# klemens-floege/oneprot

Hardware: AMD Instinct MI355X
Metric: protein-pairs/sec/node (seq+struct-token, L=512, ESM-2-150M) (higher is better)
Workload: dtype bf16; 1 GPU; cfg-2: seq<->struct_token sub-step, facebook/esm2_t30_150M_UR50D / facebook/esm2_t30_150M_UR50D, L=512, 256 pairs/GPU per modality, global batch 256, output_dim 1024, CLIP local_loss+gather_with_grad, L1 0.01, Adam 1e-3, clip 1.0, sequence encoder frozen (reference default), random-init weights; global_batch=256, seq_len=512, parallelism=dp1, frozen_sequence_encoder=True

## Files before the change

oneprot_amd/csrc/gemm_nt_ln.hip:

```cpp
#include "gemm_epi8.h"
#ifndef GLN_X_NT
#define GLN_X_NT 0
#endif

namespace gln {
using g8::gload16; using g8::lane_perm; using g8::as_f; using g8::to_rows_addr; using g8::run_groups;

constexpr int BM = 128, BN = 640, MT = 4, NT = 10, NH = 5;
constexpr int A_UNIT = BM * 128, W_UNIT = 320 * 64;
constexpr int NA = 2, NW = 6;
constexpr int OFF_W = NA * A_UNIT, OFF_S = OFF_W + NW * W_UNIT, LDS = OFF_S + 4096;
constexpr int A_IPW = 2;
static_assert(LDS <= 160 * 1024, "LDS");

struct LnArgs {
  const bf16_t* A; const unsigned char* Wp;
  int M, K, lda;
  const float* bias; const float* resid; float* x_out;
  const float* gamma; const float* beta; float eps;
  bf16_t* h_out; float* mean; float* rstd;
  int tiles;
  int late_ticks;
};

__device__ __forceinline__ void bar() { asm volatile("s_barrier" ::: "memory"); }
template <int N> __device__ __forceinline__ void wait_lgkm() { asm volatile("s_waitcnt lgkmcnt(%0)" ::"n"(N) : "memory"); }
__device__ __forceinline__ void glds16(unsigned voff, const unsigned char* sbase, unsigned lds_dst) {
  unsigned keep;
  asm volatile("s_mov_b32 %0, m0\n\ts_mov_b32 m0, %3\n\ts_nop 0\n\tglobal_load_lds_dwordx4 %1, %2\n\ts_mov_b32 m0, %0"
               : "=&s"(keep) : "v"(voff), "s"(sbase), "s"(lds_dst) : "memory");
}

template <int IMM> __device__ __forceinline__ void gload16s(u32x4& d, unsigned voff, const void* sbase) {
  asm volatile("global_load_dwordx4 %0, %1, %2 offset:%3" : "=v"(d) : "v"(voff), "s"(sbase), "n"(IMM) : "memory");
}

__global__ void __launch_bounds__(256) k_pack_w(const bf16_t* __restrict__ W, int K, u32x4* __restrict__ Wp) {
  const int units = K / 32 * 2;
  for (int idx = blockIdx.x * 256 + threadIdx.x; idx < units * 320 * 4; idx += gridDim.x * 256) {
    const int pos = idx & 3, hr = (idx >> 2) % 320, u = idx / (320 * 4);
    const int k32 = u >> 1, nh = u & 1;
    const int c = pos ^ ((hr >> 1) & 3);
    const int n = (hr / 80) * 160 + nh * 80 + hr % 80;
    Wp[idx] = *reinterpret_cast<const u32x4*>(W + (size_t)n * K + k32 * 32 + c * 8);
  }
}

__global__ void __launch_bounds__(512, 2) k_gemm_ln(const LnArgs p) {
  extern __shared__ __attribute__((aligned(16))) unsigned char smem[];
  const int tid = threadIdx.x, lane = tid & 63;
  const int wave = __builtin_amdgcn_readfirstlane(tid >> 6);
  const int grp = wave >> 2;
  const int wm = wave >> 2, wc = wave & 3;
  const int nk = p.K >> 6;
  const int PH = 4 * nk;
  const int G = gridDim.x;
  const int Q = p.tiles > (int)blockIdx.x ? (p.tiles - (int)blockIdx.x + G - 1) / G : 0;
  if (Q == 0) return;
  const unsigned lds0 = (unsigned)(uintptr_t)LDS_PTR(smem);

  const int sr = lane >> 3, sc = lane & 7;
  unsigned a_voff[A_IPW];
#pragma unroll
  for (int i = 0; i < A_IPW; ++i) {
    const int row = (i * 8 + wave) * 8 + sr;
    a_voff[i] = (unsigned)row * (unsigned)p.lda * 2u + (unsigned)(sc ^ ((row >> 1) & 7)) * 16u;
  }
  const unsigned w_voff = (unsigned)lane * 16u;
  auto issue_a = [&](const unsigned char* abase, int slot) {
#pragma unroll
    for (int i = 0; i < A_IPW; ++i) glds16(a_voff[i], abase, lds0 + slot * A_UNIT + (i * 8 + wave) * 1024);
  };
  auto issue_w = [&](const unsigned char* wbase, int slot) {
#pragma unroll
    for (int i = 0; i < 3; ++i)
      if (i < 2 || wave < 4) glds16(w_voff, wbase + (i * 8 + wave) * 1024, lds0 + OFF_W + slot * W_UNIT + (i * 8 + wave) * 1024);
  };

  int wq = 0, wu = 0, wslot = 0;
  int aq = 0, as = 0, aslot = 0;
  auto a_ptr = [&](int q, int s) { return reinterpret_cast<const unsigned char*>(p.A + (size_t)(((int)blockIdx.x + q * G) * BM) * p.lda) + (size_t)s * 128; };
  auto next_w = [&]() { if (wq < Q) issue_w(p.Wp + (size_t)wu * W_UNIT, wslot); if (++wu == PH) { wu = 0; ++wq; } wslot = wslot + 1 == NW ? 0 : wslot + 1; };
  auto next_a = [&]() { if (aq < Q) issue_a(a_ptr(aq, as), aslot); if (++as == nk) { as = 0; ++aq; } aslot ^= 1; };

  const int fr = lane & 15, fq = lane >> 4;
  const unsigned a_rd = (unsigned)(wm * 64 + fr) * 128u + (unsigned)((fq ^ (fr >> 1)) << 4);
  const unsigned w_rd = OFF_W + (unsigned)(wc * 80 + fr) * 64u + (unsigned)((fq ^ ((fr >> 1) & 3)) << 4);

  f32x4 acc[MT][NT];
  auto zero_acc = [&]() {
    float z = 0.f;
    asm volatile("" : "+v"(z));
#pragma unroll
    for (int i = 0; i < MT; ++i)
#pragma unroll
      for (int j = 0; j < NT; ++j) acc[i][j] = (f32x4){z, z, z, z};
  };
  zero_acc();
  bf8_t fa[MT], fb[NH];

  constexpr int N0 = 4 * 3 + A_IPW, N1 = 4 * 2 + A_IPW;
  int rslot = 0;
  auto phase = [&](auto kkc, auto halfc, int abuf, const bool stores_behind, const bool more) {
    constexpr int KK = decltype(kkc)::value, HALF = decltype(halfc)::value;
    if constexpr (HALF == 0) {
      const unsigned char* ab = smem + abuf * A_UNIT;
#pragma unroll
      for (int mt = 0; mt < MT; ++mt) fa[mt] = *reinterpret_cast<const bf8_t*>(ab + ((a_rd + mt * 2048) ^ (KK << 6)));
      __builtin_amdgcn_sched_barrier(0);
    }
    const unsigned char* wb = smem + rslot * W_UNIT;
#pragma unroll
    for (int nt = 0; nt < NH; ++nt) fb[nt] = *reinterpret_cast<const bf8_t*>(wb + w_rd + nt * 1024);
    __builtin_amdgcn_sched_barrier(0);
    next_w();
    if constexpr (KK == 1 && HALF == 1) next_a();
    wait_lgkm<0>();
    if (!more) wait_vmcnt<0>();
    else if (stores_behind) wait_vmcnt<63>();
    else if (grp == 0) wait_vmcnt<N0>(); else wait_vmcnt<N1>();
    bar();
    __builtin_amdgcn_sched_barrier(0);
    __builtin_amdgcn_s_setprio(1);
#pragma unroll
    for (int mt = 0; mt < MT; ++mt)
#pragma unroll
      for (int nt = 0; nt < NH; ++nt)
        acc[mt][HALF * NH + nt] = __builtin_amdgcn_mfma_f32_16x16x32_bf16(fb[nt], fa[mt], acc[mt][HALF * NH + nt], 0, 0, 0);
    __builtin_amdgcn_s_setprio(0);
    __builtin_amdgcn_sched_barrier(0);
    bar();
    rslot = rslot + 1 == NW ? 0 : rslot + 1;
  };

  next_a();
  for (int i = 0; i < 5; ++i) next_w();
  next_a();
  if (Q * nk < 2) wait_vmcnt<0>();
  else if (grp == 0) wait_vmcnt<N0>(); else wait_vmcnt<N1>();
  bar();

  const int c = lane & 15, q4 = lane >> 4;
  const int rsr = lane >> 2, rsq = lane & 3;
  const int pa = to_rows_addr(lane);
  float* scratch = reinterpret_cast<float*>(smem + OFF_S);
  int abuf = 0;
  long done_phases = 0;
  const long total_phases = (long)Q * PH;
#pragma clang loop unroll(disable)
  for (int q = 0; q < Q; ++q) {
    if (grp == 1) bar();
#pragma clang loop unroll(disable)
    for (int s = 0; s < nk; ++s) {
      const bool sb = q > 0 && s == 0;
      phase(std::integral_constant<int, 0>{}, std::integral_constant<int, 0>{}, abuf, sb, done_phases + 6 <= total_phases); ++done_phases;
      phase(std::integral_constant<int, 0>{}, std::integral_constant<int, 1>{}, abuf, sb, done_phases + 6 <= total_phases); ++done_phases;
      phase(std::integral_constant<int, 1>{}, std::integral_constant<int, 0>{}, abuf, sb, done_phases + 6 <= total_phases); ++done_phases;
      phase(std::integral_constant<int, 1>{}, std::integral_constant<int, 1>{}, abuf, sb, done_phases + 6 <= total_phases); ++done_phases;
      abuf ^= 1;
    }
    if (grp == 0) bar();

    const int m0 = ((int)blockIdx.x + q * G) * BM;
    const size_t o0 = (size_t)(m0 + wm * 64 + rsr) * BN + wc * 160 + rsq * 4;
    const size_t rstep = (size_t)16 * BN;
    const unsigned bias_off = (unsigned)(wc * 160 + q4 * 4) * 4u;
    const unsigned row_off = (unsigned)((wm * 64 + rsr) * BN + wc * 160 + rsq * 4) * 4u;
    const float* res_t = p.resid + (size_t)m0 * BN;
    float* xo = p.x_out + o0;
    float s1[MT] = {0.f, 0.f, 0.f, 0.f};
    {
      constexpr int GL = 2 + 4, GS = 4, NG = (NT / 2) * (MT / 2);
      auto load = [&](auto gc, u32x4 (&r)[GL]) {
        constexpr int g = decltype(gc)::value, a2 = 2 * (g / (MT / 2)), i2 = 2 * (g % (MT / 2));
        gload16s<a2 * 64>(r[0], bias_off, p.bias);
        gload16s<(a2 + 1) * 64>(r[1], bias_off, p.bias);
        gload16s<a2 * 64>(r[2], row_off, res_t + i2 * rstep);
        gload16s<(a2 + 1) * 64>(r[3], row_off, res_t + i2 * rstep);
        gload16s<a2 * 64>(r[4], row_off, res_t + (i2 + 1) * rstep);
        gload16s<(a2 + 1) * 64>(r[5], row_off, res_t + (i2 + 1) * rstep);
      };
      auto finish = [&](auto gc, const u32x4 (&r)[GL]) {
        constexpr int g = decltype(gc)::value, a2 = 2 * (g / (MT / 2)), i2 = 2 * (g % (MT / 2));
        float h0, h1, h2, h3;
        g8::static_for([&](auto uc) {
          constexpr int u = decltype(uc)::value, j = a2 + (u & 1), i = i2 + (u >> 1);
          u32x4 a;
          a.x = __builtin_bit_cast(unsigned, acc[i][j][0] + as_f(r[u & 1].x)); a.y = __builtin_bit_cast(unsigned, acc[i][j][1] + as_f(r[u & 1].y));
          a.z = __builtin_bit_cast(unsigned, acc[i][j][2] + as_f(r[u & 1].z)); a.w = __builtin_bit_cast(unsigned, acc[i][j][3] + as_f(r[u & 1].w));
          a = lane_perm(pa, a);
          const u32x4 t = r[2 + u];
          const float x0 = as_f(a.x) + as_f(t.x), x1 = as_f(a.y) + as_f(t.y), x2 = as_f(a.z) + as_f(t.z), x3 = as_f(a.w) + as_f(t.w);
          acc[i][j] = (f32x4){x0, x1, x2, x3};
          s1[i] += (x0 + x1) + (x2 + x3);
          if constexpr ((u & 1) == 0) { h0 = x0; h1 = x1; h2 = x2; h3 = x3; }
          else {
            __builtin_amdgcn_sched_barrier(0);
            gst(xo + i * rstep + (j - 1) * 16, h0, h1, h2, h3, GLN_X_NT);
            gst(xo + i * rstep + j * 16, x0, x1, x2, x3, GLN_X_NT);
            __builtin_amdgcn_sched_barrier(0);
          }
        }, std::make_integer_sequence<int, 4>{});
      };
      run_groups<NG, GL, GS>(load, finish);
    }
    float mw[MT], m2[MT];
#pragma unroll
    for (int i = 0; i < MT; ++i) {
      float s = s1[i];
      s += __shfl_xor(s, 1, 64); s += __shfl_xor(s, 2, 64);
      mw[i] = s * (1.0f / 160.0f);
      float qv = 0.f;
#pragma unroll
      for (int j = 0; j < NT; ++j) {
        const float a = acc[i][j][0] - mw[i], b = acc[i][j][1] - mw[i], cc = acc[i][j][2] - mw[i], d = acc[i][j][3] - mw[i];
        qv += (a * a + b * b) + (cc * cc + d * d);
      }
      qv += __shfl_xor(qv, 1, 64); qv += __shfl_xor(qv, 2, 64);
      m2[i] = qv;
      if (rsq == 0) *reinterpret_cast<float2*>(scratch + ((wm * 64 + i * 16 + rsr) * 4 + wc) * 2) = make_float2(mw[i], qv);
    }
    asm volatile("s_waitcnt lgkmcnt(0)" ::: "memory");
    bar();
    float mean[MT], rstd[MT];
#pragma unroll
    for (int i = 0; i < MT; ++i) {
      const float4 p01 = *reinterpret_cast<const float4*>(scratch + (wm * 64 + i * 16 + rsr) * 8);
      const float4 p23 = *reinterpret_cast<const float4*>(scratch + (wm * 64 + i * 16 + rsr) * 8 + 4);
      const float mu = ((p01.x + p01.z) + (p23.x + p23.z)) * 0.25f;
      const float d0 = p01.x - mu, d1 = p01.z - mu, d2 = p23.x - mu, d3 = p23.z - mu;
      const float M2 = ((p01.y + p01.w) + (p23.y + p23.w)) + 160.0f * ((d0 * d0 + d1 * d1) + (d2 * d2 + d3 * d3));
      mean[i] = mu;
      rstd[i] = rsqrtf(M2 * (1.0f / 640.0f) + p.eps);
      if (wc == 0 && rsq == 0) {
        if (p.mean) p.mean[m0 + wm * 64 + i * 16 + rsr] = mu;
        if (p.rstd) p.rstd[m0 + wm * 64 + i * 16 + rsr] = rstd[i];
      }
    }
    asm volatile("s_waitcnt lgkmcnt(0)" ::: "memory");
    bar();
    {
      constexpr int GL = 4, GS = MT, NG = NT / 2;
      const unsigned gb_off = (unsigned)(wc * 160 + rsq * 4) * 4u;
      bf16_t* ho = p.h_out + (size_t)(m0 + wm * 64 + rsr) * BN + wc * 160 + (rsq & 1) * 16 + (rsq >> 1) * 8;
      const bool odd = (rsq & 1) != 0;
      auto pass2 = [&](auto oddc) {
        constexpr bool ODDW = decltype(oddc)::value;
        auto load = [&](auto gc, u32x4 (&r)[GL]) {
          constexpr int g = decltype(gc)::value, j = 2 * (ODDW ? g : (g + NG - 1) % NG);
          gload16s<j * 64>(r[0], gb_off, p.gamma); gload16s<j * 64>(r[1], gb_off, p.beta);
          gload16s<(j + 1) * 64>(r[2], gb_off, p.gamma); gload16s<(j + 1) * 64>(r[3], gb_off, p.beta);
        };
        auto finish = [&](auto gc, const u32x4 (&r)[GL]) {
          constexpr int g = decltype(gc)::value, a = ODDW ? g : (g + NG - 1) % NG, j = 2 * a;
#pragma unroll
          for (int i = 0; i < MT; ++i) {
            u32x2 w[2];
#pragma unroll
            for (int t = 0; t < 2; ++t) {
              const u32x4 ga = r[2 * t], be = r[2 * t + 1];
              const float h0 = (acc[i][j + t][0] - mean[i]) * rstd[i] * as_f(ga.x) + as_f(be.x), h1 = (acc[i][j + t][1] - mean[i]) * rstd[i] * as_f(ga.y) + as_f(be.y);
              const float h2 = (acc[i][j + t][2] - mean[i]) * rstd[i] * as_f(ga.z) + as_f(be.z), h3 = (acc[i][j + t][3] - mean[i]) * rstd[i] * as_f(ga.w) + as_f(be.w);
              w[t].x = pack2bf(h0, h1); w[t].y = pack2bf(h2, h3);
            }
            const unsigned sx = odd ? w[0].x : w[1].x, sy = odd ? w[0].y : w[1].y;
            const unsigned rx = (unsigned)__builtin_amdgcn_update_dpp(0, (int)sx, 0xB1, 0xF, 0xF, false);
            const unsigned ry = (unsigned)__builtin_amdgcn_update_dpp(0, (int)sy, 0xB1, 0xF, 0xF, false);
            u32x4 o;
            o.x = odd ? rx : w[0].x; o.y = odd ? ry : w[0].y; o.z = odd ? w[1].x : rx; o.w = odd ? w[1].y : ry;
            gst(reinterpret_cast<u32x4*>(ho + i * rstep + a * 32), o, 0);
          }
        };
        run_groups<NG, GL, GS>(load, finish);
      };
      if (wc & 1) pass2(std::true_type{}); else pass2(std::false_type{});
    }
    zero_acc();
  }
}


namespace g1 {
constexpr int BM = 64, NWU = 3;
constexpr int A_UNIT = BM * 128;
constexpr int OFF_W = NA * A_UNIT, OFF_S = OFF_W + NWU * W_UNIT, LDS = OFF_S + 2048;
static_assert(2 * LDS <= 160 * 1024, "two work-groups per CU");
}

__global__ void __launch_bounds__(256, 2) k_gemm_ln4(const LnArgs p) {
  extern __shared__ __attribute__((aligned(16))) unsigned char smem[];
  const int tid = threadIdx.x, lane = tid & 63;
  const int wave = __builtin_amdgcn_readfirstlane(tid >> 6);
  const int wc = wave;
  const int nk = p.K >> 6;
  const int PH = 4 * nk;
  const int G = gridDim.x;
  const int Q = p.tiles > (int)blockIdx.x ? (p.tiles - (int)blockIdx.x + G - 1) / G : 0;
  if (Q == 0) return;
  const unsigned lds0 = (unsigned)(uintptr_t)LDS_PTR(smem);
  if (p.late_ticks > 0 && (int)blockIdx.x >= (G >> 1)) {
    const long long t0 = (long long)__builtin_amdgcn_s_memrealtime();
    while ((long long)__builtin_amdgcn_s_memrealtime() - t0 < p.late_ticks) __builtin_amdgcn_s_sleep(16);
  }

  const int sr = lane >> 3, sc = lane & 7;
  unsigned a_voff[2];
#pragma unroll
  for (int i = 0; i < 2; ++i) {
    const int row = (i * 4 + wave) * 8 + sr;
    a_voff[i] = (unsigned)row * (unsigned)p.lda * 2u + (unsigned)(sc ^ ((row >> 1) & 7)) * 16u;
  }
  const unsigned w_voff = (unsigned)lane * 16u;
  auto issue_a = [&](const unsigned char* abase, int slot) {
#pragma unroll
    for (int i = 0; i < 2; ++i) glds16(a_voff[i], abase, lds0 + slot * g1::A_UNIT + (i * 4 + wave) * 1024);
  };
  auto issue_w = [&](const unsigned char* wbase, int slot) {
#pragma unroll
    for (int i = 0; i < 5; ++i) glds16(w_voff, wbase + (i * 4 + wave) * 1024, lds0 + g1::OFF_W + slot * W_UNIT + (i * 4 + wave) * 1024);
  };
  int wq = 0, wu = 0, wslot = 0;
  int aq = 0, as = 0, aslot = 0;
  auto a_ptr = [&](int q, int s) { return reinterpret_cast<const unsigned char*>(p.A + (size_t)(((int)blockIdx.x + q * G) * g1::BM) * p.lda) + (size_t)s * 128; };
  auto next_w = [&]() { if (wq < Q) issue_w(p.Wp + (size_t)wu * W_UNIT, wslot); if (++wu == PH) { wu = 0; ++wq; } wslot = wslot + 1 == g1::NWU ? 0 : wslot + 1; };
  auto next_a = [&]() { if (aq < Q) issue_a(a_ptr(aq, as), aslot); if (++as == nk) { as = 0; ++aq; } aslot ^= 1; };

  const int fr = lane & 15, fq = lane >> 4;
  const unsigned a_rd = (unsigned)fr * 128u + (unsigned)((fq ^ (fr >> 1)) << 4);
  const unsigned w_rd = g1::OFF_W + (unsigned)(wc * 80 + fr) * 64u + (unsigned)((fq ^ ((fr >> 1) & 3)) << 4);

  f32x4 acc[MT][NT];
  auto zero_acc = [&]() {
    float z = 0.f;
    asm volatile("" : "+v"(z));
#pragma unroll
    for (int i = 0; i < MT; ++i)
#pragma unroll
      for (int j = 0; j < NT; ++j) acc[i][j] = (f32x4){z, z, z, z};
  };
  zero_acc();
  bf8_t fa[MT], fb[NH];

  int rslot = 0;
  bool skip_w = false;
  auto phase = [&](auto kkc, auto halfc, int abuf, const int tail, const bool a_too) {
    constexpr int KK = decltype(kkc)::value, HALF = decltype(halfc)::value;
    if constexpr (HALF == 0) {
      const unsigned char* ab = smem + abuf * g1::A_UNIT;
#pragma unroll
      for (int mt = 0; mt < MT; ++mt) fa[mt] = *reinterpret_cast<const bf8_t*>(ab + ((a_rd + mt * 2048) ^ (KK << 6)));
    }
    const unsigned char* wb = smem + rslot * W_UNIT;
#pragma unroll
    for (int nt = 0; nt < NH; ++nt) fb[nt] = *reinterpret_cast<const bf8_t*>(wb + w_rd + nt * 1024);
    __builtin_amdgcn_sched_barrier(0);
    if (!skip_w) next_w();
    skip_w = false;
    if (a_too) next_a();
    wait_lgkm<0>();
    __builtin_amdgcn_sched_barrier(0);
    __builtin_amdgcn_s_setprio(1);
#pragma unroll
    for (int mt = 0; mt < MT; ++mt)
#pragma unroll
      for (int nt = 0; nt < NH; ++nt)
        acc[mt][HALF * NH + nt] = __builtin_amdgcn_mfma_f32_16x16x32_bf16(fb[nt], fa[mt], acc[mt][HALF * NH + nt], 0, 0, 0);
    __builtin_amdgcn_s_setprio(0);
    __builtin_amdgcn_sched_barrier(0);
    if (tail == 2) wait_vmcnt<0>();
    else if (tail == 1) wait_vmcnt<63>();
    else if (KK == HALF) wait_vmcnt<5 + 2>(); else wait_vmcnt<5>();
    bar();
    rslot = rslot + 1 == g1::NWU ? 0 : rslot + 1;
  };

  next_a(); next_w(); next_w(); next_a();
  if (Q * nk < 2) wait_vmcnt<0>(); else wait_vmcnt<5 + 2>();
  bar();

  const int c = lane & 15, q4 = lane >> 4;
  const int rsr = lane >> 2, rsq = lane & 3;
  const int pa = to_rows_addr(lane);
  float* scratch = reinterpret_cast<float*>(smem + g1::OFF_S);
  int abuf = 0;
  long done = 0;
  const long total = (long)Q * PH;
  int behind = 0;
#pragma clang loop unroll(disable)
  for (int q = 0; q < Q; ++q) {
#pragma clang loop unroll(disable)
    for (int s = 0; s < nk; ++s) {
      auto tl = [&]() { const int t = done + 8 > total ? 2 : (behind > 0 ? 1 : 0); if (behind > 0) --behind; ++done; return t; };
      { const int t = tl(); phase(std::integral_constant<int, 0>{}, std::integral_constant<int, 0>{}, abuf, t, false); }
      { const int t = tl(); phase(std::integral_constant<int, 0>{}, std::integral_constant<int, 1>{}, abuf, t, false); }
      { const int t = tl(); phase(std::integral_constant<int, 1>{}, std::integral_constant<int, 0>{}, abuf, t, false); }
      { const int t = tl(); phase(std::integral_constant<int, 1>{}, std::integral_constant<int, 1>{}, abuf, t, true); }
      abuf ^= 1;
    }
    if (q + 1 < Q) { next_w(); skip_w = true; behind = 2; }

    const int m0 = ((int)blockIdx.x + q * G) * g1::BM;
    const size_t o0 = (size_t)(m0 + rsr) * BN + wc * 160 + rsq * 4;
    const size_t rstep = (size_t)16 * BN;
    const unsigned bias_off = (unsigned)(wc * 160 + q4 * 4) * 4u;
    const unsigned row_off = (unsigned)(rsr * BN + wc * 160 + rsq * 4) * 4u;
    const float* res_t = p.resid + (size_t)m0 * BN;
    float* xo = p.x_out + o0;
    float s1[MT] = {0.f, 0.f, 0.f, 0.f};
    {
      constexpr int GL = 2 + 4, GS = 4, NG = (NT / 2) * (MT / 2);
      auto load = [&](auto gc, u32x4 (&r)[GL]) {
        constexpr int g = decltype(gc)::value, a2 = 2 * (g / (MT / 2)), i2 = 2 * (g % (MT / 2));
        gload16s<a2 * 64>(r[0], bias_off, p.bias);
        gload16s<(a2 + 1) * 64>(r[1], bias_off, p.bias);
        gload16s<a2 * 64>(r[2], row_off, res_t + i2 * rstep);
        gload16s<(a2 + 1) * 64>(r[3], row_off, res_t + i2 * rstep);
        gload16s<a2 * 64>(r[4], row_off, res_t + (i2 + 1) * rstep);
        gload16s<(a2 + 1) * 64>(r[5], row_off, res_t + (i2 + 1) * rstep);
      };
      auto finish = [&](auto gc, const u32x4 (&r)[GL]) {
        constexpr int g = decltype(gc)::value, a2 = 2 * (g / (MT / 2)), i2 = 2 * (g % (MT / 2));
        float h0, h1, h2, h3;
        g8::static_for([&](auto uc) {
          constexpr int u = decltype(uc)::value, j = a2 + (u & 1), i = i2 + (u >> 1);
          u32x4 a;
          a.x = __builtin_bit_cast(unsigned, acc[i][j][0] + as_f(r[u & 1].x)); a.y = __builtin_bit_cast(unsigned, acc[i][j][1] + as_f(r[u & 1].y));
          a.z = __builtin_bit_cast(unsigned, acc[i][j][2] + as_f(r[u & 1].z)); a.w = __builtin_bit_cast(unsigned, acc[i][j][3] + as_f(r[u & 1].w));
          a = lane_perm(pa, a);
          const u32x4 t = r[2 + u];
          const float x0 = as_f(a.x) + as_f(t.x), x1 = as_f(a.y) + as_f(t.y), x2 = as_f(a.z) + as_f(t.z), x3 = as_f(a.w) + as_f(t.w);
          acc[i][j] = (f32x4){x0, x1, x2, x3};
          s1[i] += (x0 + x1) + (x2 + x3);
          if constexpr ((u & 1) == 0) { h0 = x0; h1 = x1; h2 = x2; h3 = x3; }
          else {
            __builtin_amdgcn_sched_barrier(0);
            gst(xo + i * rstep + (j - 1) * 16, h0, h1, h2, h3, GLN_X_NT);
            gst(xo + i * rstep + j * 16, x0, x1, x2, x3, GLN_X_NT);
            __builtin_amdgcn_sched_barrier(0);
          }
        }, std::make_integer_sequence<int, 4>{});
      };
      run_groups<NG, GL, GS>(load, finish);
    }
    float mw[MT], m2[MT];
#pragma unroll
    for (int i = 0; i < MT; ++i) {
      float s = s1[i];
      s += __shfl_xor(s, 1, 64); s += __shfl_xor(s, 2, 64);
      mw[i] = s * (1.0f / 160.0f);
      float qv = 0.f;
#pragma unroll
      for (int j = 0; j < NT; ++j) {
        const float a = acc[i][j][0] - mw[i], b = acc[i][j][1] - mw[i], cc = acc[i][j][2] - mw[i], d = acc[i][j][3] - mw[i];
        qv += (a * a + b * b) + (cc * cc + d * d);
      }
      qv += __shfl_xor(qv, 1, 64); qv += __shfl_xor(qv, 2, 64);
      m2[i] = qv;
      if (rsq == 0) *reinterpret_cast<float2*>(scratch + ((i * 16 + rsr) * 4 + wc) * 2) = make_float2(mw[i], qv);
    }
    asm volatile("s_waitcnt lgkmcnt(0)" ::: "memory");
    bar();
    float mean[MT], rstd[MT];
#pragma unroll
    for (int i = 0; i < MT; ++i) {
      const float4 p01 = *reinterpret_cast<const float4*>(scratch + (i * 16 + rsr) * 8);
      const float4 p23 = *reinterpret_cast<const float4*>(scratch + (i * 16 + rsr) * 8 + 4);
      const float mu = ((p01.x + p01.z) + (p23.x + p23.z)) * 0.25f;
      const float d0 = p01.x - mu, d1 = p01.z - mu, d2 = p23.x - mu, d3 = p23.z - mu;
      const float M2 = ((p01.y + p01.w) + (p23.y + p23.w)) + 160.0f * ((d0 * d0 + d1 * d1) + (d2 * d2 + d3 * d3));
      mean[i] = mu;
      rstd[i] = rsqrtf(M2 * (1.0f / 640.0f) + p.eps);
      if (wc == 0 && rsq == 0) {
        if (p.mean) p.mean[m0 + i * 16 + rsr] = mu;
        if (p.rstd) p.rstd[m0 + i * 16 + rsr] = rstd[i];
      }
    }
    asm volatile("s_waitcnt lgkmcnt(0)" ::: "memory");
    bar();
    {
      constexpr int GL = 4, GS = MT, NG = NT / 2;
      const unsigned gb_off = (unsigned)(wc * 160 + rsq * 4) * 4u;
      bf16_t* ho = p.h_out + (size_t)(m0 + rsr) * BN + wc * 160 + (rsq & 1) * 16 + (rsq >> 1) * 8;
      const bool odd = (rsq & 1) != 0;
      auto pass2 = [&](auto oddc) {
        constexpr bool ODDW = decltype(oddc)::value;
        auto load = [&](auto gc, u32x4 (&r)[GL]) {
          constexpr int g = decltype(gc)::value, j = 2 * (ODDW ? g : (g + NG - 1) % NG);
          gload16s<j * 64>(r[0], gb_off, p.gamma); gload16s<j * 64>(r[1], gb_off, p.beta);
          gload16s<(j + 1) * 64>(r[2], gb_off, p.gamma); gload16s<(j + 1) * 64>(r[3], gb_off, p.beta);
        };
        auto finish = [&](auto gc, const u32x4 (&r)[GL]) {
          constexpr int g = decltype(gc)::value, a = ODDW ? g : (g + NG - 1) % NG, j = 2 * a;
#pragma unroll
          for (int i = 0; i < MT; ++i) {
            u32x2 w[2];
#pragma unroll
            for (int t = 0; t < 2; ++t) {
              const u32x4 ga = r[2 * t], be = r[2 * t + 1];
              const float h0 = (acc[i][j + t][0] - mean[i]) * rstd[i] * as_f(ga.x) + as_f(be.x), h1 = (acc[i][j + t][1] - mean[i]) * rstd[i] * as_f(ga.y) + as_f(be.y);
              const float h2 = (acc[i][j + t][2] - mean[i]) * rstd[i] * as_f(ga.z) + as_f(be.z), h3 = (acc[i][j + t][3] - mean[i]) * rstd[i] * as_f(ga.w) + as_f(be.w);
              w[t].x = pack2bf(h0, h1); w[t].y = pack2bf(h2, h3);
            }
            const unsigned sx = odd ? w[0].x : w[1].x, sy = odd ? w[0].y : w[1].y;
            const unsigned rx = (unsigned)__builtin_amdgcn_update_dpp(0, (int)sx, 0xB1, 0xF, 0xF, false);
            const unsigned ry = (unsigned)__builtin_amdgcn_update_dpp(0, (int)sy, 0xB1, 0xF, 0xF, false);
            u32x4 o;
            o.x = odd ? rx : w[0].x; o.y = odd ? ry : w[0].y; o.z = odd ? w[1].x : rx; o.w = odd ? w[1].y : ry;
            gst(reinterpret_cast<u32x4*>(ho + i * rstep + a * 32), o, 0);
          }
        };
        run_groups<NG, GL, GS>(load, finish);
      };
      if (wc & 1) pass2(std::true_type{}); else pass2(std::false_type{});
    }
    zero_acc();
  }
}

}

extern "C" int oneprot_gemm_ln_pack_weight(const void* W, void* Wp, int N, int K, void* stream) {
  if (!W || !Wp || N != gln::BN || K <= 0 || (K & 63) || (((uintptr_t)W | (uintptr_t)Wp) & 15)) return OP_EINVAL;
  const int n = K / 32 * 2 * 320 * 4;
  int blocks = (n + 255) / 256; if (blocks > 2048) blocks = 2048;
  hipLaunchKernelGGL(gln::k_pack_w, dim3(blocks), dim3(256), 0, (hipStream_t)stream, (const bf16_t*)W, K, (u32x4*)Wp);
  return launch_status();
}

static int g_gln_form = 0;
extern "C" void oneprot_gemm_ln_form(int form) { g_gln_form = form; }
extern "C" int oneprot_gemm_ln_form_get(void) { return g_gln_form; }

extern "C" int oneprot_gemm_bf16_nt_resid_ln(const void* A, const void* Wp, int64_t M, int N, int K, int lda, const float* bias, const float* resid, float* x_out,
                                             const float* gamma, const float* beta, float eps, void* h_out, float* mean, float* rstd, void* stream) {
  if (!A || !Wp || !bias || !resid || !x_out || !gamma || !beta || !h_out || M <= 0 || M > 0x7fffffff) return OP_EINVAL;
  if (N != gln::BN || (M % gln::BM) || K <= 0 || (K & 63) || (lda & 7) || lda < K || (size_t)gln::BM * lda * 2 >= (1ull << 31)) return OP_EINVAL;
  if (((uintptr_t)A | (uintptr_t)Wp | (uintptr_t)bias | (uintptr_t)resid | (uintptr_t)x_out | (uintptr_t)gamma | (uintptr_t)beta | (uintptr_t)h_out) & 15) return OP_EINVAL;
  static bool configured = false;
  static int n_cu = 0;
  if (!configured) {
    if (hipFuncSetAttribute((const void*)gln::k_gemm_ln, hipFuncAttributeMaxDynamicSharedMemorySize, gln::LDS) != hipSuccess) return OP_ELAUNCH;
    if (hipFuncSetAttribute((const void*)gln::k_gemm_ln4, hipFuncAttributeMaxDynamicSharedMemorySize, gln::g1::LDS) != hipSuccess) return OP_ELAUNCH;
    int dev = 0; hipDeviceProp_t prop;
    if (hipGetDevice(&dev) != hipSuccess || hipGetDeviceProperties(&prop, dev) != hipSuccess) return OP_ELAUNCH;
    n_cu = prop.multiProcessorCount;
    configured = true;
  }
  gln::LnArgs a;
  a.A = (const bf16_t*)A; a.Wp = (const unsigned char*)Wp; a.M = (int)M; a.K = K; a.lda = lda; a.bias = bias; a.resid = resid; a.x_out = x_out;
  a.gamma = gamma; a.beta = beta; a.eps = eps; a.h_out = (bf16_t*)h_out; a.mean = mean; a.rstd = rstd;
  a.late_ticks = (g_gln_form >> 8) * 100;
  if ((g_gln_form & 255) == 1) {
    a.tiles = (int)(M / gln::g1::BM);
    const int grid = a.tiles < 2 * n_cu ? a.tiles : 2 * n_cu;
    hipLaunchKernelGGL(gln::k_gemm_ln4, dim3(grid), dim3(256), gln::g1::LDS, (hipStream_t)stream, a);
  } else {
    a.tiles = (int)(M / gln::BM);
    const int grid = a.tiles < n_cu ? a.tiles : n_cu;
    hipLaunchKernelGGL(gln::k_gemm_ln, dim3(grid), dim3(512), gln::LDS, (hipStream_t)stream, a);
  }
  return launch_status();
}
```

Before: 1187 protein-pairs/sec/node.

## Restructure GEMM+LayerNorm epilogue to per-wave row ownership via LDS staging

Replaces the fragment-distributed LayerNorm epilogue of the 128-row fused GEMM with a row-owner scheme. Accumulator tiles are staged through a free weight LDS slot so each wave owns whole rows, and residual loads are prefetched a few groups ahead. Bias, gamma and beta are cached once in LDS. The small-tile kernel also switches to an exact two-pass mean/variance with an extra barrier. This is meant to cut scattered global loads and cross-wave reductions, at the cost of more LDS traffic, 16 serialized barrier rounds per tile and extra LDS space.

```diff
diff --git a/oneprot_amd/csrc/gemm_nt_ln.hip b/oneprot_amd/csrc/gemm_nt_ln.hip
--- a/oneprot_amd/csrc/gemm_nt_ln.hip
+++ b/oneprot_amd/csrc/gemm_nt_ln.hip
@@ -3,13 +3,20 @@
 #define GLN_X_NT 0
 #endif
 
+#ifndef GLN_RESID_AHEAD
+#define GLN_RESID_AHEAD 2
+#endif
+#ifndef GLN_ROW_OWNER
+#define GLN_ROW_OWNER 1
+#endif
+
 namespace gln {
 using g8::gload16; using g8::lane_perm; using g8::as_f; using g8::to_rows_addr; using g8::run_groups;
 
 constexpr int BM = 128, BN = 640, MT = 4, NT = 10, NH = 5;
 constexpr int A_UNIT = BM * 128, W_UNIT = 320 * 64;
 constexpr int NA = 2, NW = 6;
-constexpr int OFF_W = NA * A_UNIT, OFF_S = OFF_W + NW * W_UNIT, LDS = OFF_S + 4096;
+constexpr int OFF_W = NA * A_UNIT, OFF_S = OFF_W + NW * W_UNIT, LDS = OFF_S + (GLN_ROW_OWNER ? 8192 : 4096);
 constexpr int A_IPW = 2;
 static_assert(LDS <= 160 * 1024, "LDS");
 
@@ -44,6 +51,26 @@
     const int n = (hr / 80) * 160 + nh * 80 + hr % 80;
     Wp[idx] = *reinterpret_cast<const u32x4*>(W + (size_t)n * K + k32 * 32 + c * 8);
   }
+}
+
+constexpr int younger_ops(int g, int ahead, int ng, int gl, int gs) {
+  int n = 0;
+  if (g < ahead) n += (ahead - 1 - g) * gl;
+  for (int s = (g < ahead ? 0 : g - ahead + 1); s < g; ++s) n += gs + (s + ahead < ng ? gl : 0);
+  return n;
+}
+
+__device__ __forceinline__ float ln_sum4(f32x4 v) { return (v[0] + v[1]) + (v[2] + v[3]); }
+__device__ __forceinline__ float ln_sq4(f32x4 v, float m) {
+#pragma clang fp contract(off)
+  const float a = v[0] - m, b = v[1] - m, cc = v[2] - m, d = v[3] - m;
+  return __builtin_fmaf(a, a, b * b) + __builtin_fmaf(cc, cc, d * d);
+}
+__device__ __forceinline__ float ln_mean(float total) { return total * (1.0f / 640.0f); }
+__device__ __forceinline__ float ln_rstd(float M2, float eps) { return rsqrtf(__builtin_fmaf(M2, 1.0f / 640.0f, eps)); }
+__device__ __forceinline__ float ln_h(float x, float mu, float rs, float ga, float be) {
+#pragma clang fp contract(off)
+  return __builtin_fmaf((x - mu) * rs, ga, be);
 }
 
 __global__ void __launch_bounds__(512, 2) k_gemm_ln(const LnArgs p) {
@@ -133,6 +160,14 @@
     rslot = rslot + 1 == NW ? 0 : rslot + 1;
   };
 
+#if GLN_ROW_OWNER
+  if (tid < BN / 4) {
+#pragma unroll
+    for (int t = 0; t < 3; ++t)
+      *reinterpret_cast<u32x4*>(smem + OFF_S + t * (BN * 4) + tid * 16) = reinterpret_cast<const u32x4*>(t == 0 ? p.bias : t == 1 ? p.gamma : p.beta)[tid];
+  }
+  wait_lgkm<0>();
+#endif
   next_a();
   for (int i = 0; i < 5; ++i) next_w();
   next_a();
@@ -162,6 +197,120 @@
     if (grp == 0) bar();
 
     const int m0 = ((int)blockIdx.x + q * G) * BM;
+#if GLN_ROW_OWNER
+    {
+      unsigned char* sl = smem + OFF_W + (rslot == 0 ? NW - 1 : rslot - 1) * W_UNIT;
+      const unsigned char* par = smem + OFF_S;
+      int ln = lane;
+      asm volatile("" : "+v"(ln));
+      const int c = ln & 15, q4 = ln >> 4;
+      const unsigned voff = (unsigned)ln * 16u, hoff = (unsigned)ln * 8u;
+      const bool tail = ln < 32;
+      const unsigned wr_off = (unsigned)(c & 7) * (BN * 4), wswz = (unsigned)((c & 3) << 2);
+      const unsigned rd_off = (unsigned)wave * (BN * 4), rswz = (unsigned)((wave & 3) << 2);
+      const float* rl = p.resid + (size_t)(m0 + wave) * BN;
+      float* xp = p.x_out + (size_t)(m0 + wave) * BN;
+      bf16_t* hp = p.h_out + (size_t)(m0 + wave) * BN;
+      constexpr int GL = 3, GS = 6, NG = BM / 8;
+      constexpr int AHEAD = GLN_RESID_AHEAD;
+      u32x4 r[AHEAD][GL];
+      auto load = [&](u32x4 (&rr)[GL]) {
+        gload16s<0>(rr[0], voff, rl);
+        gload16s<1024>(rr[1], voff, rl);
+        if (tail) gload16s<2048>(rr[2], voff, rl);
+        rl += 8 * BN;
+        asm volatile("" : "+s"(rl));
+      };
+#pragma unroll
+      for (int a = 0; a < AHEAD; ++a) load(r[a]);
+      float mean_k = 0.f, rstd_k = 0.f;
+      unsigned char* rowb = sl + rd_off;
+      unsigned char* rdw = rowb + ((((unsigned)ln) ^ rswz) << 4);
+      const unsigned char* rd = rdw;
+      g8::static_for([&](auto gc) {
+        constexpr int g = decltype(gc)::value, i = (g & 7) >> 1;
+        if (wm == (g >> 3) && (c >> 3) == (g & 1)) {
+          unsigned wz = wswz;
+          asm volatile("" : "+v"(wz));
+#pragma unroll
+          for (int j = 0; j < NT; ++j) *reinterpret_cast<f32x4*>(sl + wr_off + (((unsigned)(wc * 40 + j * 4 + q4)) ^ wz) * 16u) = acc[i][j];
+        }
+        wait_lgkm<0>();
+        bar();
+        f32x4 x[GL];
+#pragma unroll
+        for (int k = 0; k < GL; ++k) x[k] = *reinterpret_cast<const f32x4*>(rd + k * 1024);
+        constexpr int younger = younger_ops(g, AHEAD, NG, GL, GS);
+        g8::wait_vm_pin<younger>(r[g % AHEAD]);
+        const u32x4 (&t)[GL] = r[g % AHEAD];
+#pragma unroll
+        for (int k = 0; k < GL; ++k) {
+          const f32x4 pb = *reinterpret_cast<const f32x4*>(par + voff + k * 1024);
+          x[k] = (f32x4){(x[k][0] + pb[0]) + as_f(t[k].x), (x[k][1] + pb[1]) + as_f(t[k].y), (x[k][2] + pb[2]) + as_f(t[k].z), (x[k][3] + pb[3]) + as_f(t[k].w)};
+        }
+        __builtin_amdgcn_sched_barrier(0);
+        g8::gst16_s<0, GLN_X_NT != 0>(xp, voff, __builtin_bit_cast(u32x4, x[0]));
+        g8::gst16_s<1024, GLN_X_NT != 0>(xp, voff, __builtin_bit_cast(u32x4, x[1]));
+        if (tail) g8::gst16_s<2048, GLN_X_NT != 0>(xp, voff, __builtin_bit_cast(u32x4, x[2]));
+        *reinterpret_cast<f32x4*>(rdw) = x[0];
+        *reinterpret_cast<f32x4*>(rdw + 1024) = x[1];
+        if (tail) *reinterpret_cast<f32x4*>(rdw + 2048) = x[2];
+        float mw = 0.f, qw = 0.f;
+        if (ln < 16) {
+          unsigned lp = (unsigned)((ln >> 2) * 40 + (ln & 3));
+          asm volatile("" : "+v"(lp));
+          auto quad = [](float v) {
+            v += __builtin_bit_cast(float, __builtin_amdgcn_update_dpp(0, __builtin_bit_cast(int, v), 0xB1, 0xF, 0xF, false));
+            v += __builtin_bit_cast(float, __builtin_amdgcn_update_dpp(0, __builtin_bit_cast(int, v), 0x4E, 0xF, 0xF, false));
+            return v;
+          };
+          auto lane_i = [](float v, int l) { return __builtin_bit_cast(float, __builtin_amdgcn_readlane(__builtin_bit_cast(int, v), l)); };
+          auto chunk = [&](int j) { return *reinterpret_cast<const f32x4*>(rowb + (((lp + 4 * j) ^ rswz) << 4)); };
+          float s1 = 0.f;
+#pragma unroll
+          for (int j = 0; j < NT; ++j) {
+            s1 += ln_sum4(chunk(j));
+            if (j == 4) __builtin_amdgcn_sched_barrier(0);
+          }
+          s1 = quad(s1);
+          mw = ln_mean((lane_i(s1, 0) + lane_i(s1, 4)) + (lane_i(s1, 8) + lane_i(s1, 12)));
+          __builtin_amdgcn_sched_barrier(0);
+          float q1 = 0.f;
+#pragma unroll
+          for (int j = 0; j < NT; ++j) {
+            q1 += ln_sq4(chunk(j), mw);
+            if (j == 4) __builtin_amdgcn_sched_barrier(0);
+          }
+          qw = quad(q1);
+        }
+        wait_lgkm<0>();
+        bar();
+        __builtin_amdgcn_sched_barrier(0);
+        auto lane_f = [](float v, int l) { return __builtin_bit_cast(float, __builtin_amdgcn_readlane(__builtin_bit_cast(int, v), l)); };
+        const float mu = lane_f(mw, 0);
+        const float rs = ln_rstd((lane_f(qw, 0) + lane_f(qw, 4)) + (lane_f(qw, 8) + lane_f(qw, 12)), p.eps);
+        asm volatile("s_nop 3\n\tv_writelane_b32 %0, %2, %4\n\tv_writelane_b32 %1, %3, %4" : "+v"(mean_k), "+v"(rstd_k)
+                     : "s"(__builtin_amdgcn_readfirstlane(__builtin_bit_cast(int, mu))), "s"(__builtin_amdgcn_readfirstlane(__builtin_bit_cast(int, rs))), "n"(g));
+        __builtin_amdgcn_sched_barrier(0);
+        g8::static_for([&](auto kc) {
+          constexpr int k = decltype(kc)::value;
+          const f32x4 ga = *reinterpret_cast<const f32x4*>(par + 2560 + voff + k * 1024), be = *reinterpret_cast<const f32x4*>(par + 5120 + voff + k * 1024);
+          u32x2 ho;
+          ho.x = pack2bf(ln_h(x[k][0], mu, rs, ga[0], be[0]), ln_h(x[k][1], mu, rs, ga[1], be[1]));
+          ho.y = pack2bf(ln_h(x[k][2], mu, rs, ga[2], be[2]), ln_h(x[k][3], mu, rs, ga[3], be[3]));
+          if (k < 2 || tail) g8::gst8_s<k * 512>(hp, hoff, ho);
+        }, std::make_integer_sequence<int, GL>{});
+        xp += 8 * BN; hp += 8 * BN;
+        asm volatile("" : "+s"(xp), "+s"(hp));
+        if constexpr (g + AHEAD < NG) load(r[g % AHEAD]);
+        __builtin_amdgcn_sched_barrier(0);
+      }, std::make_integer_sequence<int, NG>{});
+      if (ln < NG) {
+        if (p.mean) p.mean[m0 + 8 * ln + wave] = mean_k;
+        if (p.rstd) p.rstd[m0 + 8 * ln + wave] = rstd_k;
+      }
+    }
+#else
     const size_t o0 = (size_t)(m0 + wm * 64 + rsr) * BN + wc * 160 + rsq * 4;
     const size_t rstep = (size_t)16 * BN;
     const unsigned bias_off = (unsigned)(wc * 160 + q4 * 4) * 4u;
@@ -275,6 +424,7 @@
       };
       if (wc & 1) pass2(std::true_type{}); else pass2(std::false_type{});
     }
+#endif
     zero_acc();
   }
 }
@@ -442,36 +592,35 @@
       };
       run_groups<NG, GL, GS>(load, finish);
     }
-    float mw[MT], m2[MT];
+    float mean[MT], rstd[MT];
 #pragma unroll
     for (int i = 0; i < MT; ++i) {
       float s = s1[i];
       s += __shfl_xor(s, 1, 64); s += __shfl_xor(s, 2, 64);
-      mw[i] = s * (1.0f / 160.0f);
-      float qv = 0.f;
-#pragma unroll
-      for (int j = 0; j < NT; ++j) {
-        const float a = acc[i][j][0] - mw[i], b = acc[i][j][1] - mw[i], cc = acc[i][j][2] - mw[i], d = acc[i][j][3] - mw[i];
-        qv += (a * a + b * b) + (cc * cc + d * d);
-      }
-      qv += __shfl_xor(qv, 1, 64); qv += __shfl_xor(qv, 2, 64);
-      m2[i] = qv;
-      if (rsq == 0) *reinterpret_cast<float2*>(scratch + ((i * 16 + rsr) * 4 + wc) * 2) = make_float2(mw[i], qv);
+      if (rsq == 0) scratch[((i * 16 + rsr) * 4 + wc) * 2] = s;
     }
     asm volatile("s_waitcnt lgkmcnt(0)" ::: "memory");
     bar();
-    float mean[MT], rstd[MT];
 #pragma unroll
     for (int i = 0; i < MT; ++i) {
       const float4 p01 = *reinterpret_cast<const float4*>(scratch + (i * 16 + rsr) * 8);
       const float4 p23 = *reinterpret_cast<const float4*>(scratch + (i * 16 + rsr) * 8 + 4);
-      const float mu = ((p01.x + p01.z) + (p23.x + p23.z)) * 0.25f;
-      const float d0 = p01.x - mu, d1 = p01.z - mu, d2 = p23.x - mu, d3 = p23.z - mu;
-      const float M2 = ((p01.y + p01.w) + (p23.y + p23.w)) + 160.0f * ((d0 * d0 + d1 * d1) + (d2 * d2 + d3 * d3));
-      mean[i] = mu;
-      rstd[i] = rsqrtf(M2 * (1.0f / 640.0f) + p.eps);
+      mean[i] = ln_mean((p01.x + p01.z) + (p23.x + p23.z));
+      float qv = 0.f;
+#pragma unroll
+      for (int j = 0; j < NT; ++j) qv += ln_sq4(acc[i][j], mean[i]);
+      qv += __shfl_xor(qv, 1, 64); qv += __shfl_xor(qv, 2, 64);
+      if (rsq == 0) scratch[((i * 16 + rsr) * 4 + wc) * 2 + 1] = qv;
+    }
+    asm volatile("s_waitcnt lgkmcnt(0)" ::: "memory");
+    bar();
+#pragma unroll
+    for (int i = 0; i < MT; ++i) {
+      const float4 p01 = *reinterpret_cast<const float4*>(scratch + (i * 16 + rsr) * 8);
+      const float4 p23 = *reinterpret_cast<const float4*>(scratch + (i * 16 + rsr) * 8 + 4);
+      rstd[i] = ln_rstd((p01.y + p01.w) + (p23.y + p23.w), p.eps);
       if (wc == 0 && rsq == 0) {
-        if (p.mean) p.mean[m0 + i * 16 + rsr] = mu;
+        if (p.mean) p.mean[m0 + i * 16 + rsr] = mean[i];
         if (p.rstd) p.rstd[m0 + i * 16 + rsr] = rstd[i];
       }
     }
@@ -497,8 +646,8 @@
 #pragma unroll
             for (int t = 0; t < 2; ++t) {
               const u32x4 ga = r[2 * t], be = r[2 * t + 1];
-              const float h0 = (acc[i][j + t][0] - mean[i]) * rstd[i] * as_f(ga.x) + as_f(be.x), h1 = (acc[i][j + t][1] - mean[i]) * rstd[i] * as_f(ga.y) + as_f(be.y);
-              const float h2 = (acc[i][j + t][2] - mean[i]) * rstd[i] * as_f(ga.z) + as_f(be.z), h3 = (acc[i][j + t][3] - mean[i]) * rstd[i] * as_f(ga.w) + as_f(be.w);
+              const float h0 = ln_h(acc[i][j + t][0], mean[i], rstd[i], as_f(ga.x), as_f(be.x)), h1 = ln_h(acc[i][j + t][1], mean[i], rstd[i], as_f(ga.y), as_f(be.y));
+              const float h2 = ln_h(acc[i][j + t][2], mean[i], rstd[i], as_f(ga.z), as_f(be.z)), h3 = ln_h(acc[i][j + t][3], mean[i], rstd[i], as_f(ga.w), as_f(be.w));
               w[t].x = pack2bf(h0, h1); w[t].y = pack2bf(h2, h3);
             }
             const unsigned sx = odd ? w[0].x : w[1].x, sy = odd ? w[0].y : w[1].y;
```

Result: no change. 1187 protein-pairs/sec/node (median of 3 runs) (+0.0%).
